# tingyu215/VACNIC

Hardware: AMD Instinct MI355X
Metric: train samples/sec, BART-large + CLIP ViT-L/14 full VACNIC step, GoodNews-shaped batch (higher is better)
Workload: dtype bf16

## Files before the change

vacnic_amd/csrc/gemm.hip:

```cpp
#include "gemm_kernel.h"
#include <vector>

using namespace vacgemm;

namespace {

template <int MR, int CW, int KW>
__global__ __launch_bounds__(64 * KW) void gemm_skinny_kernel(GemmP p) {
  const int lane = threadIdx.x & 63;
  const int kw = KW == 1 ? 0 : __builtin_amdgcn_readfirstlane(threadIdx.x >> 6);
  const int n0 = blockIdx.x * CW;
  constexpr int NV = MR * CW;
  float acc[NV];
#pragma unroll
  for (int i = 0; i < NV; ++i) acc[i] = 0.f;
  const int nchunk = p.K >> 3;
#pragma unroll 4
  for (int ch = lane + 64 * kw; ch < nchunk; ch += 64 * KW) {
    float wv[CW][8];
#pragma unroll
    for (int c = 0; c < CW; ++c) {
      if (n0 + c < p.N) load8bf(p.w + (size_t)(n0 + c) * p.ldw + ch * 8, wv[c]);
      else {
#pragma unroll
// ... 178 lines not shown
      const size_t off = (size_t)m * p.ldo + n;
      if (p.out_mode == 0) ((bf16_t*)p.out)[off] = f2bf(v);
      else ((float*)p.out)[off] = v;
    }
  }
}

}

extern "C" int vacnic_gemv_ln_bf16(const vacnic_gemv_ln_args* a, void* stream) {
  VPLAN_REC_STRUCT(vacnic_gemv_ln_bf16, a, stream);
  VCHECK(a && a->x && a->residual && a->gamma && a->beta && a->w && a->out, VACNIC_BAD_SHAPE, "gemv_ln: null operand");
  VCHECK(a->M >= 1 && a->M <= 8 && a->N > 0, VACNIC_UNSUPPORTED, "gemv_ln: 1 <= M <= 8 rows");
  VCHECK(a->K > 0 && (a->K & 7) == 0 && a->K <= 1024, VACNIC_UNSUPPORTED, "gemv_ln: K %% 8 == 0 and K <= 1024 (one LayerNorm row per wave)");
  VCHECK((a->ldw & 7) == 0 && a->ldw >= a->K && aligned16(a->x) && aligned16(a->residual) && aligned16(a->w), VACNIC_MISALIGNED,
         "gemv_ln: 16-byte aligned operands, ldw %% 8 == 0");
  VCHECK(a->out_mode == 0 || a->out_mode == 1, VACNIC_BAD_DTYPE, "gemv_ln: out_mode 0 (bf16) or 1 (f32)");
  VCHECK(a->ldo >= a->N, VACNIC_BAD_SHAPE, "gemv_ln: ldo < N");
  GemvLnP p;
  p.x = (const bf16_t*)a->x; p.res = (const bf16_t*)a->residual; p.gamma = a->gamma; p.beta = a->beta; p.ln_out = (bf16_t*)a->ln_out;
  p.w = (const bf16_t*)a->w; p.bias = a->bias; p.out = a->out;
  p.M = (int)a->M; p.N = (int)a->N; p.K = (int)a->K; p.ldw = (int)a->ldw; p.ldo = (int)a->ldo; p.act = a->act; p.out_mode = a->out_mode;
  p.eps = a->eps;
  constexpr int CW = 4;
  const dim3 grid((unsigned)((a->N + CW - 1) / CW));
  if (a->K <= 512) hipLaunchKernelGGL((gemv_ln_kernel<8, CW, 1>), grid, dim3(64), 0, (hipStream_t)stream, p);
  else hipLaunchKernelGGL((gemv_ln_kernel<8, CW, 2>), grid, dim3(64), 0, (hipStream_t)stream, p);
  VLAUNCH_CHECK();
  return VACNIC_OK;
}

struct TileCfg { int bm, bn, slots, per_cu; double eff; int hint; };
static const TileCfg kCfgs[3] = {
    {256, 256, 256, 1, 1.00, 256},
    {128, 128, 512, 2, 0.80, 128},
    {64, 128, 256, 1, 0.42, 64},
};
static const double kFixedUnits = 27e6;

static double cfg_cost(const TileCfg& c, int64_t M, int64_t N, int64_t kper, int64_t z) {
  const int64_t tiles = ((M + c.bm - 1) / c.bm) * ((N + c.bn - 1) / c.bn) * z;
  const int64_t rounds = (tiles + c.slots - 1) / c.slots;
  return (double)rounds * ((double)c.per_cu * c.bm * c.bn * (double)kper / c.eff + kFixedUnits);
}

static int gemm_one(const vacnic_gemm_args* a, int hint, void* stream, int ce_mode = 0, int ce_col0 = 0, bool ce_smooth = false);

extern "C" int64_t vacnic_gemm_workspace_bytes(int64_t M, int64_t N, int64_t split_k) {
  if (M <= 0 || N <= 0 || split_k <= 1) return 0;
  const int64_t mp = (M + 255) / 256 * 256, np = (N + 255) / 256 * 256;
  return mp * np * 4 * split_k;
}
extern "C" int64_t vacnic_gemm_counters(int64_t M, int64_t N) {
  if (M <= 0 || N <= 0) return 0;
  return ((M + 63) / 64) * ((N + 127) / 128);
}

extern "C" int vacnic_gemm_bf16(const vacnic_gemm_args* a, void* stream) {
  VPLAN_REC_STRUCT(vacnic_gemm_bf16, a, stream);
  VCHECK(a && a->x && a->w && a->out, VACNIC_BAD_SHAPE, "gemm: null operand");
  VCHECK(a->M > 0 && a->N > 0 && a->K > 0, VACNIC_BAD_SHAPE, "gemm: empty problem M=%ld N=%ld K=%ld",
         (long)a->M, (long)a->N, (long)a->K);
  if (a->tile_hint != 0) return gemm_one(a, a->tile_hint, stream);
  if (a->M <= 8 && !a->x_kstrided && !a->w_kstrided && a->split_k <= 1 && !a->preact && !a->dact_src && !a->residual && !a->xsum &&
      (a->K & 7) == 0)
    return gemm_one(a, 8, stream);
  const int split = a->split_k < 1 ? 1 : a->split_k;
  int64_t kper = (a->K + split - 1) / split;
  kper = (kper + BK - 1) / BK * BK;
  const int64_t z = (a->K + kper - 1) / kper;
  int best = 0; double best_cost = 1e300;
  for (int i = 0; i < 3; ++i) {
    if (i == 0 && (a->M < 256 || a->N < 256)) continue;
    const double c = cfg_cost(kCfgs[i], a->M, a->N, kper, z);
    if (c < best_cost) { best_cost = c; best = i; }
  }
  int split_cfg = -1; int64_t m_main = 0; double split_cost = best_cost;
  for (int i = 0; i < 2; ++i) {
    const int64_t rem = a->M % kCfgs[i].bm;
    if (rem == 0 || a->M - rem < kCfgs[i].bm || (i == 0 && a->N < 256)) continue;
    const double c = cfg_cost(kCfgs[i], a->M - rem, a->N, kper, z) + cfg_cost(kCfgs[2], rem, a->N, kper, z);
    if (c < 0.85 * split_cost) { split_cost = c; split_cfg = i; m_main = a->M - rem; }
  }
  const bool fwd8 = !a->x_kstrided && !a->w_kstrided && a->drop_p == 0.f;
  auto loop_of = [&](int hint) { return hint == 256 && fwd8 ? 258 : hint; };
  if (split_cfg < 0) return gemm_one(a, loop_of(kCfgs[best].hint), stream);
  vacnic_gemm_args main_a = *a, tail_a = *a;
  main_a.M = m_main;
  tail_a.M = a->M - m_main;
  const int64_t xoff = a->x_kstrided ? m_main : m_main * a->ldx;
  tail_a.x = (const char*)a->x + xoff * 2;
  const int64_t osz = a->out_mode == 0 ? 2 : 4;
  tail_a.out = (char*)a->out + m_main * a->ldo * osz;
  if (a->preact) tail_a.preact = (char*)a->preact + m_main * a->ldo * 2;
  if (a->dact_src) tail_a.dact_src = (const char*)a->dact_src + m_main * a->ldo * 2;
  if (a->residual) tail_a.residual = (const char*)a->residual + m_main * a->ldo * 2;
  if (a->xsum) tail_a.xsum = a->xsum + m_main;
  if (int e = gemm_one(&main_a, loop_of(kCfgs[split_cfg].hint), stream)) return e;
  return gemm_one(&tail_a, kCfgs[2].hint, stream);
}

static int gemm_one(const vacnic_gemm_args* a, int tile_hint, void* stream, int ce_mode, int ce_col0, bool ce_smooth) {
  VCHECK((a->ldx & 7) == 0 && (a->ldw & 7) == 0, VACNIC_MISALIGNED, "gemm: ldx/ldw must be multiples of 8");
  VCHECK(aligned16(a->x) && aligned16(a->w), VACNIC_MISALIGNED, "gemm: x/w must be 16-byte aligned");
  VCHECK(a->out_mode >= 0 && a->out_mode <= 2, VACNIC_BAD_DTYPE, "gemm: bad out_mode %d", a->out_mode);
  const int split = a->split_k < 1 ? 1 : a->split_k;
  VCHECK(split == 1 || a->out_mode == 2 || a->workspace, VACNIC_UNSUPPORTED, "gemm: split_k needs out_mode 2 or a fix-up workspace");
  if (a->workspace && split > 1) {
    VCHECK(a->counters && aligned16(a->workspace), VACNIC_BAD_SHAPE, "gemm: the split-K fix-up needs `counters` and a 16-byte aligned workspace");
    VCHECK(a->workspace_bytes >= vacnic_gemm_workspace_bytes(a->M, a->N, split) && a->counters_len >= vacnic_gemm_counters(a->M, a->N), VACNIC_BAD_SHAPE,
           "gemm: fix-up workspace %ld B / %ld counters, need %ld B / %ld", (long)a->workspace_bytes, (long)a->counters_len,
           (long)vacnic_gemm_workspace_bytes(a->M, a->N, split), (long)vacnic_gemm_counters(a->M, a->N));
    VCHECK(tile_hint != 8 && !ce_mode, VACNIC_UNSUPPORTED, "gemm: no split-K fix-up in the skinny / cross-entropy kernels");
  }
  VCHECK(a->bias == nullptr || aligned16(a->bias), VACNIC_MISALIGNED, "gemm: bias must be 16-byte aligned");
  VCHECK(a->ldo >= a->N, VACNIC_BAD_SHAPE, "gemm: ldo < N");
  VCHECK(!a->xsum || ce_mode || (a->x_kstrided && a->w_kstrided), VACNIC_UNSUPPORTED,
         "gemm: xsum (row sums of X) is implemented for the weight-gradient layout only (x_kstrided and w_kstrided)");
  if (a->x_kstrided) VCHECK(a->ldx >= ((a->M + 7) & ~7LL), VACNIC_BAD_SHAPE, "gemm: ldx too small for K-strided X");
  else VCHECK(a->ldx >= ((a->K + 7) & ~7LL), VACNIC_BAD_SHAPE, "gemm: ldx < round_up(K, 8) for K-contiguous X");
  if (a->w_kstrided) VCHECK(a->ldw >= ((a->N + 7) & ~7LL), VACNIC_BAD_SHAPE, "gemm: ldw too small for K-strided W");
  else VCHECK(a->ldw >= ((a->K + 7) & ~7LL), VACNIC_BAD_SHAPE, "gemm: ldw < round_up(K, 8) for K-contiguous W");

  auto span = [](int64_t rows, int64_t cols, int64_t ld) { return ((rows - 1) * ld + cols) * 2; };
  const int64_t K8 = (a->K + 7) & ~7LL;
  const int64_t xb = a->x_kstrided ? span(a->K, (a->M + 7) & ~7LL, a->ldx) : span(a->M, K8, a->ldx);
  const int64_t wb = a->w_kstrided ? span(a->K, (a->N + 7) & ~7LL, a->ldw) : span(a->N, K8, a->ldw);
  VCHECK(xb < 0x7ffffff0LL && wb < 0x7ffffff0LL, VACNIC_UNSUPPORTED, "gemm: operand larger than 2 GiB");

  GemmP p;
  p.x = (const bf16_t*)a->x; p.w = (const bf16_t*)a->w; p.bias = a->bias;
  p.out = a->out; p.preact = (bf16_t*)a->preact; p.dact_src = (const bf16_t*)a->dact_src;
  p.residual = (const bf16_t*)a->residual;
  p.xsum = a->xsum;
  p.M = (int)a->M; p.N = (int)a->N; p.K = (int)a->K;
  p.ldx = (int)a->ldx; p.ldw = (int)a->ldw; p.ldo = (int)a->ldo;
  p.act = a->act; p.out_mode = ce_mode ? ce_mode : a->out_mode; p.split_k = split;
  p.ce_col0 = ce_col0;
  int kps = (int)((a->K + split - 1) / split);
  kps = (kps + BK - 1) / BK * BK;
  p.k_per_split = kps;
  const int zsplits = (int)((a->K + kps - 1) / kps);
  p.split_k = zsplits;
  p.alpha = a->alpha;
  p.x_bytes = (unsigned)xb; p.w_bytes = (unsigned)wb;
  p.tiles_m = p.tiles_n = 0;
  p.ws = (a->workspace && zsplits > 1) ? (float*)a->workspace : nullptr;
  p.cnt = p.ws ? a->counters : nullptr;
  p.drop_thr = 0; p.drop_inv = 1.f; p.drop_seed = a->drop_seed; p.drop_seed_dev = (const unsigned long long*)a->drop_seed_dev;
  if (a->drop_p != 0.f) {
    VCHECK(a->drop_p > 0.f && a->drop_p < 1.f, VACNIC_BAD_SHAPE, "gemm: drop_p must be in [0, 1)");
    VCHECK(a->out_mode == 0 && a->ldo == a->N && (a->N & 15) == 0 && !ce_mode && tile_hint != 8, VACNIC_UNSUPPORTED,
           "gemm: fused activation dropout needs a contiguous bf16 output with N %% 16 == 0 (use vacnic_dropout_bf16)");
    VCHECK((zsplits == 1 || p.ws) , VACNIC_UNSUPPORTED, "gemm: fused activation dropout with split-K needs the fix-up workspace");
    unsigned thr = (unsigned)(a->drop_p * 256.f + 0.5f);
    if (thr > 255) thr = 255;
    p.drop_thr = thr;
    p.drop_inv = 256.f / (256.f - (float)thr);
  }
  hipStream_t s = (hipStream_t)stream;
  if (tile_hint == 8) {
    VCHECK(a->M <= 8 && !a->x_kstrided && !a->w_kstrided && zsplits == 1 && !a->preact && !a->dact_src && !a->residual && !a->xsum &&
           (a->K & 7) == 0, VACNIC_UNSUPPORTED, "gemm: the skinny kernel needs M <= 8, K-contiguous operands, K %% 8 == 0 and a plain epilogue");
    constexpr int CW = 4;
    dim3 grid((unsigned)((a->N + CW - 1) / CW));
    if (a->K >= 2048 && a->N <= 8192) hipLaunchKernelGGL((gemm_skinny_kernel<8, CW, 4>), grid, dim3(256), 0, s, p);
    else hipLaunchKernelGGL((gemm_skinny_kernel<8, CW, 1>), grid, dim3(64), 0, s, p);
    VLAUNCH_CHECK();
    return VACNIC_OK;
  }
  const int force = tile_hint % 1000;
  p.debug = tile_hint / 1000;
  {
    static int env_debug = -1;
    if (env_debug < 0) { const char* e = getenv("VACNIC_GEMM_DEBUG"); env_debug = e ? atoi(e) : 0; }
    p.debug |= env_debug;
  }
  if (((a->M - 1) * a->ldo + a->N) * 2 >= 0x7ffffff0LL) p.debug |= 16;
  if ((a->preact != nullptr) + (a->dact_src != nullptr) + (a->residual != nullptr) > 1) p.debug |= 16;
  if (p.drop_thr && !a->preact && !a->dact_src) p.debug |= 16;
  const bool big = force == 256;
  const bool mid = force == 128;
  if (p.drop_thr) {
    if (big) return launch_t256d(p, a->x_kstrided, a->w_kstrided, zsplits, s);
    if (force == 264) return launch_t264d(p, a->x_kstrided, a->w_kstrided, zsplits, s);
    return launch_t64d(p, a->x_kstrided, a->w_kstrided, zsplits, s);
  }
  if (force == 260) return launch_t260(p, a->x_kstrided, a->w_kstrided, zsplits, s);
  if (force == 261) return launch_t261(p, a->x_kstrided, a->w_kstrided, zsplits, s);
  if (force == 262) return launch_t262(p, a->x_kstrided, a->w_kstrided, zsplits, s);
  if (force == 264) return launch_t264(p, a->x_kstrided, a->w_kstrided, zsplits, s);
  if (force == 258 && !ce_mode) return launch_t258(p, a->x_kstrided, a->w_kstrided, zsplits, s);
  if (ce_mode && ce_smooth) return launch_t256cels(p, a->x_kstrided, a->w_kstrided, zsplits, s);
  if (ce_mode) return launch_t256ce(p, a->x_kstrided, a->w_kstrided, zsplits, s);
  if (big) return launch_t256(p, a->x_kstrided, a->w_kstrided, zsplits, s);
  if (mid) return launch_t128(p, a->x_kstrided, a->w_kstrided, zsplits, s);
  return launch_t64(p, a->x_kstrided, a->w_kstrided, zsplits, s);
}

extern "C" int vacnic_wgrad_group(const vacnic_wgrad_job* jobs, int64_t njobs, void* stream) {
  VCHECK(jobs && njobs > 0, VACNIC_BAD_SHAPE, "wgrad_group: no jobs");
  vplan::Guard vplan_guard__;
  if (vplan::outermost()) {
    std::vector<vacnic_wgrad_job> copy__(jobs, jobs + njobs);
    vplan::push([copy__, stream]() { return vacnic_wgrad_group(copy__.data(), (int64_t)copy__.size(), stream); });
  }
  constexpr int64_t US = (int64_t)GROUP_UT * 128;
  GroupP g;
  g.nunits = 0;
  g.debug = 0;
  {
    static int env_debug = -1;
    if (env_debug < 0) { const char* e = getenv("VACNIC_GEMM_DEBUG"); env_debug = e ? atoi(e) : 0; }
    g.debug = env_debug & ~8;
  }
  auto flush = [&]() -> int {
    if (g.nunits == 0) return VACNIC_OK;
    int kmax = 0;
    for (int i = 0; i < g.nunits; ++i) kmax = g.u[i].K > kmax ? g.u[i].K : kmax;
    g.k_per_phase = (kmax + BK - 1) / BK * BK;
    g.kphase = 0;
    const int e = launch_group128(g, (hipStream_t)stream);
    g.nunits = 0;
    return e;
  };
  auto span = [](int64_t rows, int64_t cols, int64_t ld) { return ((rows - 1) * ld + cols) * 2; };
  for (int64_t j = 0; j < njobs; ++j) {
    const vacnic_wgrad_job& a = jobs[j];
    VCHECK(a.dy && a.x && a.dw, VACNIC_BAD_SHAPE, "wgrad_group: job %ld has a null operand", (long)j);
    VCHECK(a.M > 0 && a.N > 0 && a.K > 0, VACNIC_BAD_SHAPE, "wgrad_group: job %ld is empty (M=%ld N=%ld K=%ld)", (long)j, (long)a.M, (long)a.N, (long)a.K);
    VCHECK((a.lddy & 7) == 0 && (a.ldx & 7) == 0 && aligned16(a.dy) && aligned16(a.x), VACNIC_MISALIGNED,
           "wgrad_group: job %ld: dy / x rows must be 16-byte aligned (ld %% 8 == 0)", (long)j);
    VCHECK(a.lddy >= ((a.N + 7) & ~7LL) && a.ldx >= ((a.K + 7) & ~7LL) && a.lddw >= a.K, VACNIC_BAD_SHAPE,
           "wgrad_group: job %ld: leading dimension too small", (long)j);
    VCHECK((a.lddw & 3) == 0 && aligned16(a.dw), VACNIC_MISALIGNED, "wgrad_group: job %ld: dw rows must be 16-byte aligned", (long)j);
    const int64_t xb = span(a.M, (a.N + 7) & ~7LL, a.lddy), wb = span(a.M, (a.K + 7) & ~7LL, a.ldx);
    VCHECK(xb < 0x7ffffff0LL && wb < 0x7ffffff0LL, VACNIC_UNSUPPORTED, "wgrad_group: job %ld: operand larger than 2 GiB", (long)j);
    for (int64_t um0 = 0; um0 < a.N; um0 += US)
      for (int64_t un0 = 0; un0 < a.K; un0 += US) {
        GroupUnit& u = g.u[g.nunits++];
        u.x = (const bf16_t*)a.dy; u.w = (const bf16_t*)a.x; u.out = a.dw;
        u.xsum = un0 == 0 ? a.dbias : nullptr;
        u.M = (int)a.N; u.N = (int)a.K; u.K = (int)a.M;
        u.ldx = (int)a.lddy; u.ldw = (int)a.ldx; u.ldo = (int)a.lddw;
        u.um0 = (int)um0; u.un0 = (int)un0;
        u.x_bytes = (unsigned)xb; u.w_bytes = (unsigned)wb;
        if (g.nunits == GROUP_MAX_UNITS) { if (int e = flush()) return e; }
      }
  }
  return flush();
}

namespace {
__global__ __launch_bounds__(256) void ce_combine_kernel(const float* __restrict__ part, const float* __restrict__ tl,
                                                          const int64_t* __restrict__ targets, float* __restrict__ row_lse,
                                                          float* __restrict__ loss_sum, float* __restrict__ count, int R, int tiles,
                                                          int64_t ignore) {
  const int lane = threadIdx.x & 63, wave = threadIdx.x >> 6;
  const int r = blockIdx.x * 4 + wave;
  float loss = 0.f, cnt = 0.f;
  if (r < R) {
    float mx = -INFINITY, sm = 0.f;
    for (int t = lane; t < tiles; t += 64) {
      const float pm = part[((size_t)r * tiles + t) * 2], ps = part[((size_t)r * tiles + t) * 2 + 1];
      if (pm > -INFINITY) {
        const float nm = fmaxf(mx, pm);
// ... 153 lines not shown
```

vacnic_amd/csrc/gemm_kernel.h:

```cpp
#pragma once
#include "common.h"
#include <stdlib.h>

namespace vacgemm {


constexpr int BK = 64;
constexpr int OOB = 0x7ffffff0;

struct GemmP {
  const bf16_t* x; const bf16_t* w; const float* bias;
  void* out; bf16_t* preact; const bf16_t* dact_src; const bf16_t* residual;
  float* xsum;
  int M, N, K;
  int ldx, ldw, ldo;
  int act, out_mode, split_k, k_per_split;
  float alpha;
  unsigned x_bytes, w_bytes;
  int tiles_m, tiles_n;
  int ce_col0;
  unsigned drop_thr; float drop_inv; unsigned long long drop_seed; const unsigned long long* drop_seed_dev;
  float* ws;
  unsigned* cnt;
  int debug;
// ... 119 lines not shown
    float* o = (float*)p.out + off;
    f32x4 a0 = *(f32x4*)o, a1 = *(f32x4*)(o + 4);
#pragma unroll
    for (int j = 0; j < 4; ++j) { a0[j] += v[j]; a1[j] += v[4 + j]; }
    *(f32x4*)o = a0; *(f32x4*)(o + 4) = a1;
  }
}

__device__ __forceinline__ void epilogue8(const GemmP& p, float v[8], int m, int n, bool add_bias, bool vec_ok) {
  const size_t off = (size_t)m * p.ldo + n;
  const int nv = min(8, p.N - n);
  const bool vec = vec_ok && nv == 8;
  if (p.alpha != 1.0f) {
#pragma unroll
    for (int j = 0; j < 8; ++j) v[j] *= p.alpha;
  }
  if (p.bias && add_bias) {
    if (nv == 8) {
      const f32x4 b0 = *(const f32x4*)(p.bias + n), b1 = *(const f32x4*)(p.bias + n + 4);
#pragma unroll
      for (int j = 0; j < 4; ++j) { v[j] += b0[j]; v[4 + j] += b1[j]; }
    } else {
      for (int j = 0; j < nv; ++j) v[j] += p.bias[n + j];
    }
  }
  if (p.preact) {
    if (vec) store8bf(p.preact + off, v);
    else for (int j = 0; j < nv; ++j) p.preact[off + j] = f2bf(v[j]);
  }
  if (p.dact_src) {
    float d[8] = {0, 0, 0, 0, 0, 0, 0, 0};
    if (vec) load8bf(p.dact_src + off, d);
    else for (int j = 0; j < nv; ++j) d[j] = bf2f(p.dact_src[off + j]);
#pragma unroll
    for (int j = 0; j < 8; ++j) v[j] *= act_bwd(p.act, d[j]);
  } else if (p.act != VACNIC_ACT_NONE) {
#pragma unroll
    for (int j = 0; j < 8; ++j) v[j] = act_fwd(p.act, v[j]);
  }
  if (p.residual) {
    float d[8] = {0, 0, 0, 0, 0, 0, 0, 0};
    if (vec) load8bf(p.residual + off, d);
    else for (int j = 0; j < nv; ++j) d[j] = bf2f(p.residual[off + j]);
#pragma unroll
    for (int j = 0; j < 8; ++j) v[j] += d[j];
  }
  if (p.debug & 1) {
    if (v[0] == 12345.678f) ((bf16_t*)p.out)[off] = 0;
  } else if (p.out_mode == 0) {
    bf16_t* o = (bf16_t*)p.out + off;
    if (vec) store8bf(o, v);
    else for (int j = 0; j < nv; ++j) o[j] = f2bf(v[j]);
  } else if (p.out_mode == 1) {
    float* o = (float*)p.out + off;
    if (nv == 8 && (p.ldo & 3) == 0) {
      *(f32x4*)o = (f32x4){v[0], v[1], v[2], v[3]};
      *(f32x4*)(o + 4) = (f32x4){v[4], v[5], v[6], v[7]};
    } else {
      for (int j = 0; j < nv; ++j) o[j] = v[j];
    }
  } else {
    float* o = (float*)p.out + off;
    if (nv == 8 && (p.ldo & 3) == 0) {
      f32x4 a0 = *(f32x4*)o, a1 = *(f32x4*)(o + 4);
#pragma unroll
      for (int j = 0; j < 4; ++j) { a0[j] += v[j]; a1[j] += v[4 + j]; }
      *(f32x4*)o = a0; *(f32x4*)(o + 4) = a1;
    } else {
      for (int j = 0; j < nv; ++j) o[j] += v[j];
    }
  }
}

template <int V> struct IC { static constexpr int value = V; };

__device__ __forceinline__ void lds_barrier() {
  asm volatile("s_waitcnt lgkmcnt(0)" ::: "memory");
  __builtin_amdgcn_s_barrier();
  asm volatile("" ::: "memory");
}



template <int N>
__device__ __forceinline__ void wait_vm_lgkm() { asm volatile("s_waitcnt vmcnt(%0) lgkmcnt(0)" ::"n"(N) : "memory"); }

template <int FB, int FA>
__device__ __forceinline__ void p8_loop(f32x4 (&acc)[FB][FA], char* smem, __amdgpu_buffer_rsrc_t xs, __amdgpu_buffer_rsrc_t ws,
                                        int m0, int n0, int RX, int RW, int kbeg, int kend, int ntile, int ldx, int ldw,
                                        int wave, int lane) {
  static_assert(FB == 4 && FA == 8, "128 x 64 outputs per wave");
  constexpr int HALF = 16384, BUF = 4 * HALF;
  constexpr int SLOT_W0 = 0, SLOT_X0 = HALF, SLOT_W1 = 2 * HALF, SLOT_X1 = 3 * HALF;
  const int wm = wave & 1, wn = wave >> 1;
  const int sr = lane >> 2, sc = (lane & 3) ^ (((lane >> 5) & 1) << 1);
  unsigned xoff[2], woff[2];
#pragma unroll
  for (int h = 0; h < 2; ++h) {
    const int gx = m0 + (wave >> 2) * 128 + h * 64 + (wave & 3) * 16 + sr;
    const int gw = n0 + (wave >> 1) * 64 + h * 32 + (wave & 1) * 16 + sr;
    xoff[h] = gx < RX ? ((unsigned)gx * (unsigned)ldx + (unsigned)(sc * 8)) * 2u : (unsigned)OOB;
    woff[h] = gw < RW ? ((unsigned)gw * (unsigned)ldw + (unsigned)(sc * 8)) * 2u : (unsigned)OOB;
  }
  const int klim = kend - sc * 8;
  char* const sdst = smem + wave * 2048;
  auto stage = [&](__amdgpu_buffer_rsrc_t rsrc, unsigned roff, int slot, int t) {
    const int k0 = kbeg + t * 64;
    const unsigned v0 = k0 < klim ? roff + (unsigned)k0 * 2u : (unsigned)OOB;
    const unsigned v1 = k0 + 32 < klim ? roff + (unsigned)(k0 + 32) * 2u : (unsigned)OOB;
    char* d = sdst + slot;
    __builtin_amdgcn_raw_ptr_buffer_load_lds(rsrc, LDS_PTR(d), 16, (int)v0, 0, 0, 0);
    __builtin_amdgcn_raw_ptr_buffer_load_lds(rsrc, LDS_PTR(d + 1024), 16, (int)v1, 0, 0, 0);
  };
  const int fro = (lane & 15) * 64 + (((lane >> 4) ^ (((lane >> 3) & 1) << 1)) << 4);
  const char* const xrd = smem + fro + wm * 8192;
  const char* const wrd = smem + fro + wn * 4096;

  stage(ws, woff[0], SLOT_W0, 0); stage(xs, xoff[0], SLOT_X0, 0); stage(ws, woff[1], SLOT_W1, 0); stage(xs, xoff[1], SLOT_X1, 0);
  stage(ws, woff[0], BUF + SLOT_W0, 1); stage(xs, xoff[0], BUF + SLOT_X0, 1); stage(ws, woff[1], BUF + SLOT_W1, 1);
  asm volatile("s_waitcnt vmcnt(6)" ::: "memory");
  __builtin_amdgcn_sched_barrier(0);
  __builtin_amdgcn_s_barrier();
  __builtin_amdgcn_sched_barrier(0);
  const bool grp_b = wave >= 4;
  if (grp_b) { __builtin_amdgcn_sched_barrier(0); __builtin_amdgcn_s_barrier(); __builtin_amdgcn_sched_barrier(0); }

  bf16x8 xf[4][2], w0[2][2], w1[2][2];
#define VAC_P8_BAR()  __builtin_amdgcn_sched_barrier(0); __builtin_amdgcn_s_barrier(); __builtin_amdgcn_sched_barrier(0)
#define VAC_P8_MFMA(A0, B0, WF)                                                                                          \
  asm volatile("s_waitcnt lgkmcnt(0)" ::: "memory");                                                                     \
  __builtin_amdgcn_sched_barrier(0);                                                                                     \
  __builtin_amdgcn_s_setprio(1);                                                                                         \
  _Pragma("unroll") for (int kk = 0; kk < 2; ++kk)                                                                       \
    _Pragma("unroll") for (int b = 0; b < 2; ++b)                                                                        \
      _Pragma("unroll") for (int a = 0; a < 4; ++a)                                                                      \
        acc[B0 + b][A0 + a] = __builtin_amdgcn_mfma_f32_16x16x32_bf16(WF[b][kk], xf[a][kk], acc[B0 + b][A0 + a], 0, 0, 0); \
  __builtin_amdgcn_s_setprio(0);                                                                                         \
  VAC_P8_BAR()
  auto ktile = [&](auto par_c, int t) {
    constexpr int PAR = decltype(par_c)::value;
    const char* const xb = xrd + PAR * BUF;
    const char* const wb = wrd + PAR * BUF;
#pragma unroll
    for (int b = 0; b < 2; ++b)
#pragma unroll
      for (int kk = 0; kk < 2; ++kk) w0[b][kk] = *(const bf16x8*)(wb + SLOT_W0 + b * 2048 + kk * 1024);
    __builtin_amdgcn_sched_barrier(0);
#pragma unroll
    for (int a = 0; a < 4; ++a)
#pragma unroll
      for (int kk = 0; kk < 2; ++kk) xf[a][kk] = *(const bf16x8*)(xb + SLOT_X0 + a * 2048 + kk * 1024);
    __builtin_amdgcn_sched_barrier(0);
    stage(xs, xoff[1], (PAR ^ 1) * BUF + SLOT_X1, t + 1);
    asm volatile("s_waitcnt lgkmcnt(8)" ::: "memory");
    VAC_P8_BAR();
    VAC_P8_MFMA(0, 0, w0);
#pragma unroll
    for (int b = 0; b < 2; ++b)
#pragma unroll
      for (int kk = 0; kk < 2; ++kk) w1[b][kk] = *(const bf16x8*)(wb + SLOT_W1 + b * 2048 + kk * 1024);
    __builtin_amdgcn_sched_barrier(0);
    stage(ws, woff[0], PAR * BUF + SLOT_W0, t + 2);
    VAC_P8_BAR();
    VAC_P8_MFMA(0, 2, w1);
#pragma unroll
    for (int a = 0; a < 4; ++a)
#pragma unroll
      for (int kk = 0; kk < 2; ++kk) xf[a][kk] = *(const bf16x8*)(xb + SLOT_X1 + a * 2048 + kk * 1024);
    __builtin_amdgcn_sched_barrier(0);
    stage(xs, xoff[0], PAR * BUF + SLOT_X0, t + 2);
    VAC_P8_BAR();
    VAC_P8_MFMA(4, 2, w1);
    stage(ws, woff[1], PAR * BUF + SLOT_W1, t + 2);
    asm volatile("s_waitcnt vmcnt(6)" ::: "memory");
    VAC_P8_BAR();
    VAC_P8_MFMA(4, 0, w0);
  };
  for (int t = 0; t < ntile; t += 2) {
    ktile(IC<0>{}, t);
    if (t + 1 >= ntile) break;
    ktile(IC<1>{}, t + 1);
  }
#undef VAC_P8_MFMA
#undef VAC_P8_BAR
  if (!grp_b) { __builtin_amdgcn_sched_barrier(0); __builtin_amdgcn_s_barrier(); __builtin_amdgcn_sched_barrier(0); }
}

template <int BM, int BN, int WM, int WN, int BKT, int NSTAGE, bool PIPE, bool XKS, bool WKS, bool CE, bool DR = false, bool LS = false, bool P8 = false>
__device__ __forceinline__ void gemm_tile(const GemmP& p, const int m0, const int n0, const int tn, const int zsplit, const int tile_id = 0) {
  constexpr int NWAVE = WM * WN, NTHR = 64 * NWAVE;
  constexpr int TM = BM / WM, TN = BN / WN;
  constexpr int FA = TM / 16, FB = TN / 16;
  constexpr int XT = BM * BKT * 2, WT = BN * BKT * 2, STAGE = XT + WT;
  extern __shared__ __attribute__((aligned(16))) char smem[];
  const int tid = threadIdx.x;
  const int lane = tid & 63;
  const int wave = __builtin_amdgcn_readfirstlane(tid >> 6);
  const int wm = wave % WM, wn = wave / WM;
  const int kbeg = zsplit * p.k_per_split;
  const int kend = min(p.K, kbeg + p.k_per_split);
  const int ntile = (p.debug & 2) ? 0 : (kend - kbeg + BKT - 1) / BKT;

  __amdgpu_buffer_rsrc_t xs = __builtin_amdgcn_make_buffer_rsrc((void*)p.x, 0, p.x_bytes, 0x00020000);
  __amdgpu_buffer_rsrc_t ws = __builtin_amdgcn_make_buffer_rsrc((void*)p.w, 0, p.w_bytes, 0x00020000);

  const int RX = XKS ? ((p.M + 7) & ~7) : p.M;
  const int RW = WKS ? ((p.N + 7) & ~7) : p.N;

  f32x4 acc[FB][FA];
#pragma unroll
  for (int b = 0; b < FB; ++b)
#pragma unroll
    for (int a = 0; a < FA; ++a) acc[b][a] = (f32x4){0.f, 0.f, 0.f, 0.f};

  constexpr int XSN = FA / WN;
  static_assert(FA % WN == 0 && FA / WN <= 4, "xsum: row blocks split over the waves of a row group, <= 4 each");
  constexpr bool XS = XKS && WKS;
  const bool xs_on = XS && p.xsum != nullptr;
  int xs_next = tn;
  f32x4 accs = (f32x4){0.f, 0.f, 0.f, 0.f};
#define VAC_XSUM_MFMA(XF)                                                                   \
  if constexpr (XS) {                                                                       \
    _Pragma("unroll") for (int w_ = 0; w_ < WN; ++w_)                                       \
      if (wn == w_) {                                                                       \
        _Pragma("unroll") for (int i = 0; i < XSN; ++i) {                                   \
          const short o_ = (lane & 15) == i ? (short)0x3F80 : (short)0;                              \
          const bf16x8 sel_ = {o_, o_, o_, o_, o_, o_, o_, o_};                             \
          accs = __builtin_amdgcn_mfma_f32_16x16x32_bf16(sel_, XF[w_ * XSN + i], accs, 0, 0, 0); \
        }                                                                                   \
      }                                                                                     \
  }
#define VAC_XSUM(XF, STEP)                                                                  \
  if (XS && xs_on && (STEP) == xs_next) {                                                   \
    VAC_XSUM_MFMA(XF)                                                                       \
    xs_next += p.tiles_n;                                                                   \
  }

  constexpr int LOADS = (BM + BN) * BKT * 2 / 1024 / NWAVE;
  static_assert(LOADS * (NSTAGE - 2) <= 63, "vmcnt immediate");
  constexpr bool PIPED = PIPE && BKT == 64 && NSTAGE == 2 && !P8;
  constexpr int PRO = PIPED ? 2 : NSTAGE - 1;
  if constexpr (!P8) {
#pragma unroll
    for (int s = 0; s < PRO; ++s) {
      stage_tile<XKS, BM, BKT, NWAVE>(xs, smem + s * STAGE, m0, RX, kbeg + s * BKT, kend, p.ldx, wave, lane);
      stage_tile<WKS, BN, BKT, NWAVE>(ws, smem + s * STAGE + XT, n0, RW, kbeg + s * BKT, kend, p.ldw, wave, lane);
    }
    wait_vm_lgkm<LOADS * (PRO - 1)>();
    __builtin_amdgcn_s_barrier();
  }
  int cur = 0, nxt = NSTAGE - 1;
  if constexpr (P8) {
    static_assert(BM == 256 && BN == 256 && WM == 2 && WN == 4 && BKT == 64 && NSTAGE == 2 && !XKS && !WKS,
                  "8-phase loop: 256 x 256 tile, 2 x 4 waves, both operands K-contiguous");
    p8_loop(acc, smem, xs, ws, m0, n0, RX, RW, kbeg, kend, ntile, p.ldx, p.ldw, wave, lane);
  } else if constexpr (PIPE && BKT == 32 && NSTAGE == 4) {
    static_assert(NWAVE == 8 && LOADS >= 2, "ping-pong loop is written for 8 waves (two per SIMD)");
    const bool grp_b = wave >= NWAVE / 2;
    const int nst = ntile;
    bf16x8 xf[FA], wf[FB];
    if (grp_b) { __builtin_amdgcn_sched_barrier(0); __builtin_amdgcn_s_barrier(); __builtin_amdgcn_sched_barrier(0); }
    int rd = 0, wr = 3;
    for (int h = 0; h < nst; ++h) {
      const char* xr = smem + rd * STAGE;
      char* xw = smem + wr * STAGE;
      if (!(p.debug & 128) || h == 0) {
#pragma unroll
        for (int a = 0; a < FA; ++a) xf[a] = read_frag<XKS, BM, BKT>(xr, wm * TM + a * 16, 0, lane);
#pragma unroll
        for (int b = 0; b < FB; ++b) wf[b] = read_frag<WKS, BN, BKT>(xr + XT, wn * TN + b * 16, 0, lane);
      }
      if (!(p.debug & 32)) {
        stage_tile<XKS, BM, BKT, NWAVE>(xs, xw, m0, RX, kbeg + (h + 3) * BKT, kend, p.ldx, wave, lane);
        stage_tile<WKS, BN, BKT, NWAVE>(ws, xw + XT, n0, RW, kbeg + (h + 3) * BKT, kend, p.ldw, wave, lane);
      }
      wait_vm_lgkm<2 * LOADS>();
      __builtin_amdgcn_sched_barrier(0);
      __builtin_amdgcn_s_barrier();
      __builtin_amdgcn_sched_barrier(0);
      __builtin_amdgcn_s_setprio(1);
#pragma unroll
      for (int b = 0; b < FB; ++b)
#pragma unroll
        for (int a = 0; a < FA; ++a)
          acc[b][a] = __builtin_amdgcn_mfma_f32_16x16x32_bf16(wf[b], xf[a], acc[b][a], 0, 0, 0);
      VAC_XSUM(xf, h)
      __builtin_amdgcn_s_setprio(0);
      __builtin_amdgcn_sched_barrier(0);
      __builtin_amdgcn_s_barrier();
      __builtin_amdgcn_sched_barrier(0);
      rd = (rd + 1) & 3;
      wr = (wr + 1) & 3;
    }
    if (!grp_b) { __builtin_amdgcn_sched_barrier(0); __builtin_amdgcn_s_barrier(); __builtin_amdgcn_sched_barrier(0); }
  } else if constexpr (PIPED) {
    bf16x8 xf0[FA], wf0[FB], xf1[FA], wf1[FB];
#pragma unroll
    for (int a = 0; a < FA; ++a) xf0[a] = read_frag<XKS, BM, BKT>(smem, wm * TM + a * 16, 0, lane);
#pragma unroll
    for (int b = 0; b < FB; ++b) wf0[b] = read_frag<WKS, BN, BKT>(smem + XT, wn * TN + b * 16, 0, lane);
    for (int t = 0; t < ntile; ++t) {
      char* xcur = smem + cur * STAGE;
      char* wcur = xcur + XT;
#pragma unroll
      for (int a = 0; a < FA; ++a) xf1[a] = read_frag<XKS, BM, BKT>(xcur, wm * TM + a * 16, 1, lane);
#pragma unroll
      for (int b = 0; b < FB; ++b) wf1[b] = read_frag<WKS, BN, BKT>(wcur, wn * TN + b * 16, 1, lane);
#pragma unroll
      for (int b = 0; b < FB; ++b)
#pragma unroll
        for (int a = 0; a < FA; ++a)
          acc[b][a] = __builtin_amdgcn_mfma_f32_16x16x32_bf16(wf0[b], xf0[a], acc[b][a], 0, 0, 0);
      if (XS && xs_on && t == xs_next) { VAC_XSUM_MFMA(xf0) }
      asm volatile("s_waitcnt vmcnt(0) lgkmcnt(0)" ::: "memory");
      __builtin_amdgcn_s_barrier();
      stage_tile<XKS, BM, BKT, NWAVE>(xs, xcur, m0, RX, kbeg + (t + 2) * BKT, kend, p.ldx, wave, lane);
      stage_tile<WKS, BN, BKT, NWAVE>(ws, wcur, n0, RW, kbeg + (t + 2) * BKT, kend, p.ldw, wave, lane);
      cur ^= 1;
      {
        const char* xn = smem + cur * STAGE;
#pragma unroll
        for (int a = 0; a < FA; ++a) xf0[a] = read_frag<XKS, BM, BKT>(xn, wm * TM + a * 16, 0, lane);
#pragma unroll
        for (int b = 0; b < FB; ++b) wf0[b] = read_frag<WKS, BN, BKT>(xn + XT, wn * TN + b * 16, 0, lane);
      }
#pragma unroll
      for (int b = 0; b < FB; ++b)
#pragma unroll
        for (int a = 0; a < FA; ++a)
          acc[b][a] = __builtin_amdgcn_mfma_f32_16x16x32_bf16(wf1[b], xf1[a], acc[b][a], 0, 0, 0);
      VAC_XSUM(xf1, t)
    }
  } else {
  bf16x8 xf[FA], wf[FB];
  for (int t = 0; t < ntile; ++t) {
    char* xcur = smem + cur * STAGE;
    char* wcur = xcur + XT;
    if (!(p.debug & 32)) {
// ... 467 lines not shown
int launch_gemm_ce_smooth(const GemmP& p0, bool xks, bool wks, int zsplits, hipStream_t s) {
  if (xks || wks || zsplits != 1) { vacnic_set_error("gemm: the cross-entropy epilogues are built for the forward layout without split-K"); return VACNIC_UNSUPPORTED; }
  GemmP p = p0;
  p.tiles_m = (p.M + BM - 1) / BM; p.tiles_n = (p.N + BN - 1) / BN;
  constexpr size_t lds = NSTAGE * (BM + BN) * BKT * 2;
  static_assert(lds >= 64 * (BN + 4) * 4, "epilogue staging must fit in the operand buffers");
  auto kern = gemm_ce_smooth_kernel<BM, BN, WM, WN, BKT, NSTAGE, PIPE>;
  if (lds > 65536) {
    static bool once = false;
    if (!once) { (void)hipFuncSetAttribute((const void*)kern, hipFuncAttributeMaxDynamicSharedMemorySize, (int)lds); once = true; }
  }
  hipLaunchKernelGGL(kern, dim3(p.tiles_m * p.tiles_n), dim3(64 * WM * WN), lds, s, p);
  VLAUNCH_CHECK();
  return VACNIC_OK;
}

constexpr int GROUP_UT = 8;
constexpr int GROUP_MAX_UNITS = 16;
struct GroupUnit {
  const bf16_t* x; const bf16_t* w; float* out; float* xsum;
  int M, N, K, ldx, ldw, ldo;
  int um0, un0;
  unsigned x_bytes, w_bytes;
};
struct GroupP { GroupUnit u[GROUP_MAX_UNITS]; int nunits; int debug; int kphase; int k_per_phase; };

template <int BM, int BN, int WM, int WN, int BKT, int NSTAGE, bool PIPE>
__global__ __launch_bounds__(64 * WM * WN, 2) void gemm_group_kernel(GroupP g) {
  constexpr int TPU = GROUP_UT * GROUP_UT;
  const int xcd = blockIdx.x & 7, j = blockIdx.x >> 3;
  const int unit = (j / TPU) * 8 + xcd;
  if (unit >= g.nunits) return;
  const int t = j % TPU;
  const int tm = t / GROUP_UT, tn = t % GROUP_UT;
  const GroupUnit& u = g.u[unit];
  const int m0 = u.um0 + tm * BM, n0 = u.un0 + tn * BN;
  if (m0 >= u.M || n0 >= u.N || g.kphase * g.k_per_phase >= u.K) return;
  GemmP p;
  p.x = u.x; p.w = u.w; p.bias = nullptr; p.out = u.out; p.preact = nullptr; p.dact_src = nullptr; p.residual = nullptr;
  p.xsum = u.xsum;
  p.M = u.M; p.N = u.N; p.K = u.K; p.ldx = u.ldx; p.ldw = u.ldw; p.ldo = u.ldo;
  p.act = VACNIC_ACT_NONE; p.out_mode = 2; p.split_k = 1; p.k_per_split = g.k_per_phase;
  p.alpha = 1.0f; p.x_bytes = u.x_bytes; p.w_bytes = u.w_bytes;
  p.tiles_m = GROUP_UT; p.tiles_n = min(GROUP_UT, (u.N - u.un0 + BN - 1) / BN);
  p.ce_col0 = 0; p.debug = g.debug; p.ws = nullptr; p.cnt = nullptr; p.drop_thr = 0;
  gemm_tile<BM, BN, WM, WN, BKT, NSTAGE, PIPE, true, true, false>(p, m0, n0, tn, g.kphase);
}

template <int BM, int BN, int WM, int WN, int BKT, int NSTAGE, bool PIPE>
int launch_gemm_group(const GroupP& g, hipStream_t s) {
  static_assert(BM == 128 && BN == 128, "units are GROUP_UT x GROUP_UT tiles of 128 x 128");
  const int rounds = (g.nunits + 7) / 8;
  dim3 grid(rounds * 8 * GROUP_UT * GROUP_UT), block(64 * WM * WN);
  constexpr size_t lds = NSTAGE * (BM + BN) * BKT * 2;
  auto kern = gemm_group_kernel<BM, BN, WM, WN, BKT, NSTAGE, PIPE>;
  if (lds > 65536) {
    static bool once = false;
    if (!once) { (void)hipFuncSetAttribute((const void*)kern, hipFuncAttributeMaxDynamicSharedMemorySize, (int)lds); once = true; }
  }
  hipLaunchKernelGGL(kern, grid, block, lds, s, g);
  VLAUNCH_CHECK();
  return VACNIC_OK;
}


template <int BM, int BN, int WM, int WN, int BKT, int NSTAGE, bool PIPE = false, bool CE = false, bool DR = false, bool P8 = false>
int launch_gemm(const GemmP& p0, bool xks, bool wks, int zsplits, hipStream_t s) {
  GemmP p = p0;
  p.tiles_m = (p.M + BM - 1) / BM; p.tiles_n = (p.N + BN - 1) / BN;
  const int nwg = p.tiles_m * p.tiles_n * zsplits;
  dim3 grid(nwg), block(64 * WM * WN);
  constexpr size_t lds = NSTAGE * (BM + BN) * BKT * 2;
  static_assert(lds >= 64 * (BN + 4) * 4, "epilogue staging must fit in the operand buffers");
#define VAC_LAUNCH(XK, WK)                                                                            \
  do {                                                                                                \
    auto kern = gemm_kernel<BM, BN, WM, WN, BKT, NSTAGE, PIPE, XK, WK, CE, DR, P8>;                                      \
    if (lds > 65536) {                                                                                \
      static bool once = false;                                                                       \
      if (!once) { (void)hipFuncSetAttribute((const void*)kern, hipFuncAttributeMaxDynamicSharedMemorySize, (int)lds); once = true; } \
    }                                                                                                 \
    hipLaunchKernelGGL(kern, grid, block, lds, s, p);                                                 \
  } while (0)
  if constexpr (P8) {
    if (xks || wks) { vacnic_set_error("gemm: the 8-phase loop is built for the forward layout (both operands K-contiguous)"); return VACNIC_UNSUPPORTED; }
    VAC_LAUNCH(false, false);
  } else if constexpr (CE) {
    if (xks || wks) { vacnic_set_error("gemm: the cross-entropy epilogues are built for the forward layout only"); return VACNIC_UNSUPPORTED; }
    VAC_LAUNCH(false, false);
  } else if constexpr (DR) {
    if (xks) { vacnic_set_error("gemm: fused activation dropout is built for K-contiguous X (forward / dgrad layouts)"); return VACNIC_UNSUPPORTED; }
    if (wks) VAC_LAUNCH(false, true); else VAC_LAUNCH(false, false);
  } else {
    if (!xks && !wks) VAC_LAUNCH(false, false);
    else if (!xks && wks) VAC_LAUNCH(false, true);
    else if (xks && wks) VAC_LAUNCH(true, true);
    else VAC_LAUNCH(true, false);
  }
#undef VAC_LAUNCH
  VLAUNCH_CHECK();
  return VACNIC_OK;
}


int launch_t256(const GemmP& p, bool xks, bool wks, int zsplits, hipStream_t s);
int launch_t258(const GemmP& p, bool xks, bool wks, int zsplits, hipStream_t s);
int launch_t264(const GemmP& p, bool xks, bool wks, int zsplits, hipStream_t s);
int launch_t128(const GemmP& p, bool xks, bool wks, int zsplits, hipStream_t s);
int launch_t64(const GemmP& p, bool xks, bool wks, int zsplits, hipStream_t s);
int launch_t260(const GemmP& p, bool xks, bool wks, int zsplits, hipStream_t s);
int launch_t261(const GemmP& p, bool xks, bool wks, int zsplits, hipStream_t s);
int launch_t262(const GemmP& p, bool xks, bool wks, int zsplits, hipStream_t s);
int launch_t256ce(const GemmP& p, bool xks, bool wks, int zsplits, hipStream_t s);
int launch_t256cels(const GemmP& p, bool xks, bool wks, int zsplits, hipStream_t s);
int launch_t256d(const GemmP& p, bool xks, bool wks, int zsplits, hipStream_t s);
int launch_t264d(const GemmP& p, bool xks, bool wks, int zsplits, hipStream_t s);
int launch_t64d(const GemmP& p, bool xks, bool wks, int zsplits, hipStream_t s);
int launch_group128(const GroupP& g, hipStream_t s);

}
```

Measured before the change: 500.7.

## Extend 8-phase GEMM loop to dgrad layout and dropout-fused forward

Generalizes the 8-phase ping-pong main loop so the W operand can be K-strided, staging it row-wise and reading it through ds_read_b64_tr_b16 transposed LDS reads. Dgrad-layout GEMMs with 256 tiles now route to a new 259 variant. Forward GEMMs with fused dropout now use a 258 dropout variant. The aim is to give backward and dropout GEMMs the better-overlapped loop in place of the generic 256 kernel, at the cost of new address math and LDS swizzle paths that carry a correctness risk.

Result: no change. 502.4 (median of 6 runs) (+0.3%).

```diff
diff --git a/vacnic_amd/csrc/gemm.hip b/vacnic_amd/csrc/gemm.hip
--- a/vacnic_amd/csrc/gemm.hip
+++ b/vacnic_amd/csrc/gemm.hip
@@ -284,8 +284,11 @@
     const double c = cfg_cost(kCfgs[i], a->M - rem, a->N, kper, z) + cfg_cost(kCfgs[2], rem, a->N, kper, z);
     if (c < 0.85 * split_cost) { split_cost = c; split_cfg = i; m_main = a->M - rem; }
   }
-  const bool fwd8 = !a->x_kstrided && !a->w_kstrided && a->drop_p == 0.f;
-  auto loop_of = [&](int hint) { return hint == 256 && fwd8 ? 258 : hint; };
+  auto loop_of = [&](int hint) {
+    if (hint != 256 || a->x_kstrided) return hint;
+    if (!a->w_kstrided) return 258;
+    return a->drop_p == 0.f && kper <= 4096 ? 259 : hint;
+  };
   if (split_cfg < 0) return gemm_one(a, loop_of(kCfgs[best].hint), stream);
   vacnic_gemm_args main_a = *a, tail_a = *a;
   main_a.M = m_main;
@@ -383,7 +386,13 @@
   if (p.drop_thr && !a->preact && !a->dact_src) p.debug |= 16;
   const bool big = force == 256;
   const bool mid = force == 128;
+  if (force == 259) {
+    VCHECK(a->w_kstrided && !a->x_kstrided && !ce_mode && !p.drop_thr, VACNIC_UNSUPPORTED,
+           "gemm: tile_hint 259 is the 8-phase loop of the dgrad layout (w_kstrided alone, no fused dropout); forward layout: tile_hint 258");
+    return launch_t259d(p, zsplits, s);
+  }
   if (p.drop_thr) {
+    if (force == 258) return launch_t258d(p, a->x_kstrided, a->w_kstrided, zsplits, s);
     if (big) return launch_t256d(p, a->x_kstrided, a->w_kstrided, zsplits, s);
     if (force == 264) return launch_t264d(p, a->x_kstrided, a->w_kstrided, zsplits, s);
     return launch_t64d(p, a->x_kstrided, a->w_kstrided, zsplits, s);
diff --git a/vacnic_amd/csrc/gemm_kernel.h b/vacnic_amd/csrc/gemm_kernel.h
--- a/vacnic_amd/csrc/gemm_kernel.h
+++ b/vacnic_amd/csrc/gemm_kernel.h
@@ -225,10 +225,19 @@
 
 
 
+template <int OFF>
+__device__ __forceinline__ bf16x8 tr_frag_uncounted(unsigned addr) {
+  static_assert(OFF >= 0 && OFF + 1024 < 65536, "ds offset field");
+  bf16x4 lo, hi;
+  asm volatile("ds_read_b64_tr_b16 %0, %1 offset:%2" : "=v"(lo) : "v"(addr), "n"(OFF) : "memory");
+  asm volatile("ds_read_b64_tr_b16 %0, %1 offset:%2" : "=v"(hi) : "v"(addr), "n"(OFF + 1024) : "memory");
+  return __builtin_shufflevector(lo, hi, 0, 1, 2, 3, 4, 5, 6, 7);
+}
+
 template <int N>
 __device__ __forceinline__ void wait_vm_lgkm() { asm volatile("s_waitcnt vmcnt(%0) lgkmcnt(0)" ::"n"(N) : "memory"); }
 
-template <int FB, int FA>
+template <bool WKS, int FB, int FA>
 __device__ __forceinline__ void p8_loop(f32x4 (&acc)[FB][FA], char* smem, __amdgpu_buffer_rsrc_t xs, __amdgpu_buffer_rsrc_t ws,
                                         int m0, int n0, int RX, int RW, int kbeg, int kend, int ntile, int ldx, int ldw,
                                         int wave, int lane) {
@@ -243,24 +252,71 @@
     const int gx = m0 + (wave >> 2) * 128 + h * 64 + (wave & 3) * 16 + sr;
     const int gw = n0 + (wave >> 1) * 64 + h * 32 + (wave & 1) * 16 + sr;
     xoff[h] = gx < RX ? ((unsigned)gx * (unsigned)ldx + (unsigned)(sc * 8)) * 2u : (unsigned)OOB;
-    woff[h] = gw < RW ? ((unsigned)gw * (unsigned)ldw + (unsigned)(sc * 8)) * 2u : (unsigned)OOB;
+    if (!WKS) woff[h] = gw < RW ? ((unsigned)gw * (unsigned)ldw + (unsigned)(sc * 8)) * 2u : (unsigned)OOB;
   }
   const int klim = kend - sc * 8;
+  const int skr = lane >> 4, slc = (lane & 15) ^ ((skr | ((wave & 1) << 2)) << 1);
+  const int sk = wave * 8 + skr;
+  if (WKS) {
+#pragma unroll
+    for (int h = 0; h < 2; ++h) {
+      const int gw = n0 + (slc >> 2) * 64 + h * 32 + (slc & 3) * 8;
+      woff[h] = gw < RW ? ((unsigned)(kbeg + sk) * (unsigned)ldw + (unsigned)gw) * 2u : (unsigned)OOB;
+    }
+  }
+  const int kslim = kend - kbeg - sk;
   char* const sdst = smem + wave * 2048;
-  auto stage = [&](__amdgpu_buffer_rsrc_t rsrc, unsigned roff, int slot, int t) {
-    const int k0 = kbeg + t * 64;
-    const unsigned v0 = k0 < klim ? roff + (unsigned)k0 * 2u : (unsigned)OOB;
-    const unsigned v1 = k0 + 32 < klim ? roff + (unsigned)(k0 + 32) * 2u : (unsigned)OOB;
+  auto stage = [&](auto ks_c, __amdgpu_buffer_rsrc_t rsrc, unsigned roff, int ld, int slot, int t) {
+    unsigned v0, v1;
+    if constexpr (decltype(ks_c)::value) {
+      const int kt = t * 64;
+      v0 = kt < kslim ? roff + (unsigned)kt * (unsigned)ld * 2u : (unsigned)OOB;
+      v1 = kt + 4 < kslim ? roff + (unsigned)(kt + 4) * (unsigned)ld * 2u : (unsigned)OOB;
+    } else {
+      const int k0 = kbeg + t * 64;
+      v0 = k0 < klim ? roff + (unsigned)k0 * 2u : (unsigned)OOB;
+      v1 = k0 + 32 < klim ? roff + (unsigned)(k0 + 32) * 2u : (unsigned)OOB;
+    }
     char* d = sdst + slot;
     __builtin_amdgcn_raw_ptr_buffer_load_lds(rsrc, LDS_PTR(d), 16, (int)v0, 0, 0, 0);
     __builtin_amdgcn_raw_ptr_buffer_load_lds(rsrc, LDS_PTR(d + 1024), 16, (int)v1, 0, 0, 0);
   };
+  auto stage_x = [&](int h, int slot, int t) { stage(IC<false>{}, xs, xoff[h], ldx, slot, t); };
+  auto stage_w = [&](int h, int slot, int t) { stage(IC<WKS>{}, ws, woff[h], ldw, slot, t); };
   const int fro = (lane & 15) * 64 + (((lane >> 4) ^ (((lane >> 3) & 1) << 1)) << 4);
   const char* const xrd = smem + fro + wm * 8192;
   const char* const wrd = smem + fro + wn * 4096;
-
-  stage(ws, woff[0], SLOT_W0, 0); stage(xs, xoff[0], SLOT_X0, 0); stage(ws, woff[1], SLOT_W1, 0); stage(xs, xoff[1], SLOT_X1, 0);
-  stage(ws, woff[0], BUF + SLOT_W0, 1); stage(xs, xoff[0], BUF + SLOT_X0, 1); stage(ws, woff[1], BUF + SLOT_W1, 1);
+  bf16x8 xf[4][2], w0[2][2], w1[2][2];
+  unsigned wtr[2];
+  {
+    const int g = lane >> 4, q = (lane & 15) >> 2, pp = lane & 3;
+    const int k = 8 * g + q;
+    const unsigned base = (unsigned)(size_t)LDS_PTR(smem) + k * 256 + (pp & 1) * 8;
+#pragma unroll
+    for (int b = 0; b < 2; ++b) wtr[b] = base + ((((wn * 32 + b * 16) >> 3) + (pp >> 1)) ^ (fk(k) << 1)) * 16;
+  }
+  auto read_x = [&](auto slot_c, auto a_c, auto kk_c) -> bf16x8 {
+    constexpr int SLOT = decltype(slot_c)::value, A = decltype(a_c)::value, KK = decltype(kk_c)::value;
+    return *(const bf16x8*)(xrd + SLOT + A * 2048 + KK * 1024);
+  };
+  auto read_w = [&](auto slot_c, auto b_c, auto kk_c) -> bf16x8 {
+    constexpr int SLOT = decltype(slot_c)::value, B = decltype(b_c)::value, KK = decltype(kk_c)::value;
+    if constexpr (WKS) return tr_frag_uncounted<SLOT % BUF + KK * 8192>(wtr[B] + SLOT / BUF * BUF);
+    else return *(const bf16x8*)(wrd + SLOT + B * 2048 + KK * 1024);
+  };
+  auto load_w = [&](auto slot_c, bf16x8 (&wf)[2][2]) {
+    wf[0][0] = read_w(slot_c, IC<0>{}, IC<0>{}); wf[0][1] = read_w(slot_c, IC<0>{}, IC<1>{});
+    wf[1][0] = read_w(slot_c, IC<1>{}, IC<0>{}); wf[1][1] = read_w(slot_c, IC<1>{}, IC<1>{});
+  };
+  auto load_x = [&](auto slot_c) {
+    xf[0][0] = read_x(slot_c, IC<0>{}, IC<0>{}); xf[0][1] = read_x(slot_c, IC<0>{}, IC<1>{});
+    xf[1][0] = read_x(slot_c, IC<1>{}, IC<0>{}); xf[1][1] = read_x(slot_c, IC<1>{}, IC<1>{});
+    xf[2][0] = read_x(slot_c, IC<2>{}, IC<0>{}); xf[2][1] = read_x(slot_c, IC<2>{}, IC<1>{});
+    xf[3][0] = read_x(slot_c, IC<3>{}, IC<0>{}); xf[3][1] = read_x(slot_c, IC<3>{}, IC<1>{});
+  };
+
+  stage_w(0, SLOT_W0, 0); stage_x(0, SLOT_X0, 0); stage_w(1, SLOT_W1, 0); stage_x(1, SLOT_X1, 0);
+  stage_w(0, BUF + SLOT_W0, 1); stage_x(0, BUF + SLOT_X0, 1); stage_w(1, BUF + SLOT_W1, 1);
   asm volatile("s_waitcnt vmcnt(6)" ::: "memory");
   __builtin_amdgcn_sched_barrier(0);
   __builtin_amdgcn_s_barrier();
@@ -268,7 +324,6 @@
   const bool grp_b = wave >= 4;
   if (grp_b) { __builtin_amdgcn_sched_barrier(0); __builtin_amdgcn_s_barrier(); __builtin_amdgcn_sched_barrier(0); }
 
-  bf16x8 xf[4][2], w0[2][2], w1[2][2];
 #define VAC_P8_BAR()  __builtin_amdgcn_sched_barrier(0); __builtin_amdgcn_s_barrier(); __builtin_amdgcn_sched_barrier(0)
 #define VAC_P8_MFMA(A0, B0, WF)                                                                                          \
   asm volatile("s_waitcnt lgkmcnt(0)" ::: "memory");                                                                     \
@@ -282,39 +337,25 @@
   VAC_P8_BAR()
   auto ktile = [&](auto par_c, int t) {
     constexpr int PAR = decltype(par_c)::value;
-    const char* const xb = xrd + PAR * BUF;
-    const char* const wb = wrd + PAR * BUF;
-#pragma unroll
-    for (int b = 0; b < 2; ++b)
-#pragma unroll
-      for (int kk = 0; kk < 2; ++kk) w0[b][kk] = *(const bf16x8*)(wb + SLOT_W0 + b * 2048 + kk * 1024);
+    load_w(IC<PAR * BUF + SLOT_W0>{}, w0);
     __builtin_amdgcn_sched_barrier(0);
-#pragma unroll
-    for (int a = 0; a < 4; ++a)
-#pragma unroll
-      for (int kk = 0; kk < 2; ++kk) xf[a][kk] = *(const bf16x8*)(xb + SLOT_X0 + a * 2048 + kk * 1024);
+    load_x(IC<PAR * BUF + SLOT_X0>{});
     __builtin_amdgcn_sched_barrier(0);
-    stage(xs, xoff[1], (PAR ^ 1) * BUF + SLOT_X1, t + 1);
+    stage_x(1, (PAR ^ 1) * BUF + SLOT_X1, t + 1);
     asm volatile("s_waitcnt lgkmcnt(8)" ::: "memory");
     VAC_P8_BAR();
     VAC_P8_MFMA(0, 0, w0);
-#pragma unroll
-    for (int b = 0; b < 2; ++b)
-#pragma unroll
-      for (int kk = 0; kk < 2; ++kk) w1[b][kk] = *(const bf16x8*)(wb + SLOT_W1 + b * 2048 + kk * 1024);
+    load_w(IC<PAR * BUF + SLOT_W1>{}, w1);
     __builtin_amdgcn_sched_barrier(0);
-    stage(ws, woff[0], PAR * BUF + SLOT_W0, t + 2);
+    stage_w(0, PAR * BUF + SLOT_W0, t + 2);
     VAC_P8_BAR();
     VAC_P8_MFMA(0, 2, w1);
-#pragma unroll
-    for (int a = 0; a < 4; ++a)
-#pragma unroll
-      for (int kk = 0; kk < 2; ++kk) xf[a][kk] = *(const bf16x8*)(xb + SLOT_X1 + a * 2048 + kk * 1024);
+    load_x(IC<PAR * BUF + SLOT_X1>{});
     __builtin_amdgcn_sched_barrier(0);
-    stage(xs, xoff[0], PAR * BUF + SLOT_X0, t + 2);
+    stage_x(0, PAR * BUF + SLOT_X0, t + 2);
     VAC_P8_BAR();
     VAC_P8_MFMA(4, 2, w1);
-    stage(ws, woff[1], PAR * BUF + SLOT_W1, t + 2);
+    stage_w(1, PAR * BUF + SLOT_W1, t + 2);
     asm volatile("s_waitcnt vmcnt(6)" ::: "memory");
     VAC_P8_BAR();
     VAC_P8_MFMA(4, 0, w0);
@@ -394,9 +435,9 @@
   }
   int cur = 0, nxt = NSTAGE - 1;
   if constexpr (P8) {
-    static_assert(BM == 256 && BN == 256 && WM == 2 && WN == 4 && BKT == 64 && NSTAGE == 2 && !XKS && !WKS,
-                  "8-phase loop: 256 x 256 tile, 2 x 4 waves, both operands K-contiguous");
-    p8_loop(acc, smem, xs, ws, m0, n0, RX, RW, kbeg, kend, ntile, p.ldx, p.ldw, wave, lane);
+    static_assert(BM == 256 && BN == 256 && WM == 2 && WN == 4 && BKT == 64 && NSTAGE == 2 && !XKS,
+                  "8-phase loop: 256 x 256 tile, 2 x 4 waves, X K-contiguous (forward and dgrad layouts)");
+    p8_loop<WKS>(acc, smem, xs, ws, m0, n0, RX, RW, kbeg, kend, ntile, p.ldx, p.ldw, wave, lane);
   } else if constexpr (PIPE && BKT == 32 && NSTAGE == 4) {
     static_assert(NWAVE == 8 && LOADS >= 2, "ping-pong loop is written for 8 waves (two per SIMD)");
     const bool grp_b = wave >= NWAVE / 2;
@@ -1030,7 +1071,7 @@
     hipLaunchKernelGGL(kern, grid, block, lds, s, p);                                                 \
   } while (0)
   if constexpr (P8) {
-    if (xks || wks) { vacnic_set_error("gemm: the 8-phase loop is built for the forward layout (both operands K-contiguous)"); return VACNIC_UNSUPPORTED; }
+    if (xks || wks) { vacnic_set_error("gemm: tile_hint 258 is the 8-phase loop of the forward layout (both operands K-contiguous); K-strided operands: tile_hint 259"); return VACNIC_UNSUPPORTED; }
     VAC_LAUNCH(false, false);
   } else if constexpr (CE) {
     if (xks || wks) { vacnic_set_error("gemm: the cross-entropy epilogues are built for the forward layout only"); return VACNIC_UNSUPPORTED; }
@@ -1052,6 +1093,8 @@
 
 int launch_t256(const GemmP& p, bool xks, bool wks, int zsplits, hipStream_t s);
 int launch_t258(const GemmP& p, bool xks, bool wks, int zsplits, hipStream_t s);
+int launch_t258d(const GemmP& p, bool xks, bool wks, int zsplits, hipStream_t s);
+int launch_t259d(const GemmP& p, int zsplits, hipStream_t s);
 int launch_t264(const GemmP& p, bool xks, bool wks, int zsplits, hipStream_t s);
 int launch_t128(const GemmP& p, bool xks, bool wks, int zsplits, hipStream_t s);
 int launch_t64(const GemmP& p, bool xks, bool wks, int zsplits, hipStream_t s);
diff --git a/vacnic_amd/csrc/gemm_t258d.hip b/vacnic_amd/csrc/gemm_t258d.hip
--- /dev/null
+++ b/vacnic_amd/csrc/gemm_t258d.hip
@@ -0,0 +1,4 @@
+#include "gemm_kernel.h"
+namespace vacgemm {
+int launch_t258d(const GemmP& p, bool xks, bool wks, int zsplits, hipStream_t s) { return launch_gemm<256, 256, 2, 4, 64, 2, false, false, true, true>(p, xks, wks, zsplits, s); }
+}
diff --git a/vacnic_amd/csrc/gemm_t259d.hip b/vacnic_amd/csrc/gemm_t259d.hip
--- /dev/null
+++ b/vacnic_amd/csrc/gemm_t259d.hip
@@ -0,0 +1,15 @@
+#include "gemm_kernel.h"
+namespace vacgemm {
+int launch_t259d(const GemmP& p0, int zsplits, hipStream_t s) {
+  constexpr int BM = 256, BN = 256;
+  GemmP p = p0;
+  p.tiles_m = (p.M + BM - 1) / BM; p.tiles_n = (p.N + BN - 1) / BN;
+  constexpr size_t lds = 2 * (BM + BN) * 64 * 2;
+  auto kern = gemm_kernel<BM, BN, 2, 4, 64, 2, false, false, true, false, false, true>;
+  static bool once = false;
+  if (!once) { (void)hipFuncSetAttribute((const void*)kern, hipFuncAttributeMaxDynamicSharedMemorySize, (int)lds); once = true; }
+  hipLaunchKernelGGL(kern, dim3(p.tiles_m * p.tiles_n * zsplits), dim3(512), lds, s, p);
+  VLAUNCH_CHECK();
+  return VACNIC_OK;
+}
+}
```
